# LargeWorldModel/LWM

Measured on AMD Instinct MI355X. Metric: tokens/sec fwd+bwd, LWM-7B RingAttention hot path (32 layers x 32 heads x 128), higher is better.
Workload: dtype bf16 (f32 logits/softmax/accumulate)

## Files before the change

lwm_amd/csrc/attn_fwd64.h:

```cpp
#pragma once

namespace lwm {

constexpr int kF4BQ = 256;
constexpr int kF4BK = 64;
constexpr int kF4Threads = 256;
constexpr int kF4TileBytes = kF4BK * kRowBytes;
constexpr int kF4OffMeta = 4 * kF4TileBytes;
constexpr int kF4OffScan = kF4OffMeta + 3 * kF4BK * 4;
constexpr int kF4LdsBytes = kF4OffScan + 64;
#ifndef LWM_F4_AHEAD
#define LWM_F4_AHEAD 7
#endif
constexpr int kF4Ahead = LWM_F4_AHEAD;
static_assert(kF4Ahead >= 1 && kF4Ahead <= 7, "prefetch distance in fragments");
constexpr int f4_pre_gap(int j) { return 17 - 2 * kF4Ahead + 2 * j; }
constexpr int kF4G0a = 2, kF4G0b = 8, kF4G1a = 2, kF4G1b = 7, kF4G1c = 12, kF4G2a = 1, kF4G2b = 5, kF4G2c = 9;

struct F4Ctx {
    uint32_t ka[8];
    uint32_t vlo[4], vup[4];
    lds_t lds;
    int tid, lane, hi, wave;
    float thr[2];
    float mref[2];
    float nbase[2];
    float lsum[2];
    float c;
    float thr_on;
};

struct F4Stage {
    uint32_t voff_k[4], voff_v[4];
    const char* kb;
    const char* vb;
    int64_t ktile_bytes, vtile_bytes;
};

template <int N>
LWM_DEVICE void f4_dma(const uint32_t* voff, const char* src, lds_t dst) {
#ifdef LWM_EMU
    for (int j = 0; j < N; ++j) glds_load_b128(src + voff[j], dst + 4096 * j);
#else
    const uint64_t a = (uint64_t)src;
    const uint64_t u = ((uint64_t)(uint32_t)__builtin_amdgcn_readfirstlane((int)(a >> 32)) << 32) |
                       (uint32_t)__builtin_amdgcn_readfirstlane((int)a);
    unsigned keep;
    if (N == 4) {
        asm volatile(
            "s_mov_b32 %0, m0\n\ts_nop 3\n\t"
            "s_mov_b32 m0, %6\n\ts_nop 0\n\tglobal_load_lds_dwordx4 %1, %5\n\t"
            "s_add_u32 m0, m0, 0x1000\n\ts_nop 0\n\tglobal_load_lds_dwordx4 %2, %5\n\t"
            "s_add_u32 m0, m0, 0x1000\n\ts_nop 0\n\tglobal_load_lds_dwordx4 %3, %5\n\t"
            "s_add_u32 m0, m0, 0x1000\n\ts_nop 0\n\tglobal_load_lds_dwordx4 %4, %5\n\t"
            "s_mov_b32 m0, %0"
            : "=&s"(keep)
            : "v"(voff[0]), "v"(voff[1]), "v"(voff[2]), "v"(voff[3]), "s"(u), "s"(dst)
            : "memory", "scc");
    } else {
        asm volatile(
            "s_mov_b32 %0, m0\n\ts_nop 3\n\t"
            "s_mov_b32 m0, %4\n\ts_nop 0\n\tglobal_load_lds_dwordx4 %1, %3\n\t"
            "s_add_u32 m0, m0, 0x1000\n\ts_nop 0\n\tglobal_load_lds_dwordx4 %2, %3\n\t"
            "s_mov_b32 m0, %0"
            : "=&s"(keep)
            : "v"(voff[0]), "v"(voff[1]), "s"(u), "s"(dst)
            : "memory", "scc");
    }
#endif
}

LWM_DEVICE void f4_dma1(uint32_t voff, const char* src, lds_t dst) {
#ifdef LWM_EMU
    glds_load_b128(src + voff, dst);
#else
    const uint64_t a = (uint64_t)src;
    const uint64_t u = ((uint64_t)(uint32_t)__builtin_amdgcn_readfirstlane((int)(a >> 32)) << 32) |
                       (uint32_t)__builtin_amdgcn_readfirstlane((int)a);
    asm volatile("s_mov_b32 m0, %2\n\ts_nop 0\n\tglobal_load_lds_dwordx4 %0, %1" ::"v"(voff), "s"(u), "s"(dst) : "memory");
#endif
}
struct F4Dma {
    const char* k_lo_src;
    const char* k_up_src;
    const char* v_src;
    lds_t k_lo_dst, k_up_dst, v_dst;
};

LWM_DEVICE void f4_stage_offsets(const AttnParams& p, int wave, int lane, int kt, F4Stage& st) {
    const int slot = lane & 15;
    for (int j = 0; j < 4; ++j) {
        const int row = 4 * (wave + 4 * j) + (lane >> 4);
        int krow = kt * kF4BK + row;
        krow = krow < p.Sk ? krow : p.Sk - 1;
        const int rel = krow - kt * kF4BK;
        const int col = (slot ^ swz(row)) << 3;
        st.voff_k[j] = (uint32_t)(((int64_t)rel * p.k_ss + col) * 2);
        st.voff_v[j] = (uint32_t)(((int64_t)rel * p.v_ss + col) * 2);
    }
}

LWM_DEVICE void f4_meta_stage(const AttnParams& p, const F4Ctx& cx, int b, int kt, int buf) {
    if (cx.tid < kF4BK) {
        const int krow = kt * kF4BK + cx.tid;
        const int kr = krow < p.Sk ? krow : p.Sk - 1;
        const uint8_t kvalid = p.key_valid ? p.key_valid[(int64_t)b * p.Sk + kr] : (uint8_t)1;
        const int32_t kseg = p.seg_k ? p.seg_k[(int64_t)b * p.Sk + kr] : 0;
        const bool ok = krow < p.Sk && kvalid != 0;
        lds_write_i32(cx.lds + kF4OffMeta + buf * kF4BK * 4 + cx.tid * 4, ok ? kseg : kSegInvalid);
    }
}

#ifdef LWM_EMU
LWM_DEVICE void f4_mfma_s_first(f32x16& d, bf16x8 a, bf16x8 b) { d = mfma_32x32x16(a, b, zero_f32x16()); }
LWM_DEVICE void f4_mfma_s(f32x16& d, bf16x8 a, bf16x8 b) { d = mfma_32x32x16(a, b, d); }
LWM_DEVICE void f4_mfma_o(f32x16& d, bf16x8 a, bf16x8 b) { d = mfma_32x32x16(a, b, d); }
LWM_DEVICE void f4_mfma_settle() {}
LWM_DEVICE void f4_settle_s(f32x16 (&)[2]) {}
LWM_DEVICE void f4_settle_acc(f32x16 (&)[2][4]) {}
LWM_DEVICE float f4_fma(float x, float c, float d) { return fmaf(x, c, d); }
LWM_DEVICE float f4_exp2(float x) { return exp2f(x); }
LWM_DEVICE uint32_t f4_cvt_pk(float lo, float hi) { return pack_bf16x2(lo, hi); }
LWM_DEVICE void f4_add(float& acc, float x) { acc += x; }
LWM_DEVICE float f4_add2(float a, float b) { return a + b; }
LWM_DEVICE void f4_max3(float& m, float a, float b) { m = fmaxf(fmaxf(m, a), b); }
LWM_DEVICE bf16x8 f4_load_agpr(const bf16_t* g) { return __builtin_bit_cast(bf16x8, global_load_b128(g)); }
LWM_DEVICE void f4_load_agpr_wait(bf16x8 (&)[2][8]) {}
LWM_DEVICE void f4_load_agpr_wait8(bf16x8 (&)[8]) {}
LWM_DEVICE void f4_scale_acc(f32x16& d, float alpha) { d *= alpha; }
#else
LWM_DEVICE void f4_mfma_s_first(f32x16& d, bf16x8 a, bf16x8 b) {
    asm volatile("v_mfma_f32_32x32x16_bf16 %0, %1, %2, 0" : "=&v"(d) : "v"(a), "a"(b));
}
LWM_DEVICE void f4_mfma_s(f32x16& d, bf16x8 a, bf16x8 b) {
    asm volatile("v_mfma_f32_32x32x16_bf16 %0, %1, %2, %0" : "+v"(d) : "v"(a), "a"(b));
}
LWM_DEVICE void f4_mfma_o(f32x16& d, bf16x8 a, bf16x8 b) {
    asm volatile("v_mfma_f32_32x32x16_bf16 %0, %1, %2, %0" : "+a"(d) : "v"(a), "v"(b));
}
LWM_DEVICE void f4_mfma_settle() { asm volatile("s_nop 7\n\ts_nop 7"); }
LWM_DEVICE void f4_settle_s(f32x16 (&s)[2]) { asm volatile("s_nop 7\n\ts_nop 7" : "+v"(s[0]), "+v"(s[1])); }
LWM_DEVICE void f4_settle_acc(f32x16 (&a)[2][4]) {
    asm volatile("s_nop 7\n\ts_nop 7"
                 : "+a"(a[0][0]), "+a"(a[0][1]), "+a"(a[0][2]), "+a"(a[0][3]), "+a"(a[1][0]), "+a"(a[1][1]), "+a"(a[1][2]), "+a"(a[1][3]));
}
LWM_DEVICE float f4_fma(float x, float c, float d) {
    float y;
    asm volatile("v_fma_f32 %0, %1, %2, %3" : "=v"(y) : "v"(x), "v"(c), "v"(d));
    return y;
}
LWM_DEVICE float f4_exp2(float x) {
    float y;
    asm volatile("v_exp_f32 %0, %1" : "=v"(y) : "v"(x));
    return y;
}
LWM_DEVICE uint32_t f4_cvt_pk(float lo, float hi) {
    uint32_t y;
    asm volatile("v_cvt_pk_bf16_f32 %0, %1, %2" : "=v"(y) : "v"(lo), "v"(hi));
    return y;
}
LWM_DEVICE void f4_add(float& acc, float x) { asm volatile("v_add_f32 %0, %0, %1" : "+v"(acc) : "v"(x)); }
LWM_DEVICE float f4_add2(float a, float b) {
    float y;
    asm volatile("v_add_f32 %0, %1, %2" : "=v"(y) : "v"(a), "v"(b));
    return y;
}
LWM_DEVICE bf16x8 f4_load_agpr(const bf16_t* g) {
    u32x4 r;
    asm volatile("global_load_dwordx4 %0, %1, off" : "=a"(r) : "v"(g) : "memory");
    return __builtin_bit_cast(bf16x8, r);
}
LWM_DEVICE void f4_load_agpr_wait(bf16x8 (&q)[2][8]) {
    asm volatile("s_waitcnt vmcnt(0)"
                 : "+a"(q[0][0]), "+a"(q[0][1]), "+a"(q[0][2]), "+a"(q[0][3]), "+a"(q[0][4]), "+a"(q[0][5]), "+a"(q[0][6]), "+a"(q[0][7]),
                   "+a"(q[1][0]), "+a"(q[1][1]), "+a"(q[1][2]), "+a"(q[1][3]), "+a"(q[1][4]), "+a"(q[1][5]), "+a"(q[1][6]), "+a"(q[1][7])
                 :
                 : "memory");
}
LWM_DEVICE void f4_load_agpr_wait8(bf16x8 (&q)[8]) {
    asm volatile("s_waitcnt vmcnt(0)"
                 : "+a"(q[0]), "+a"(q[1]), "+a"(q[2]), "+a"(q[3]), "+a"(q[4]), "+a"(q[5]), "+a"(q[6]), "+a"(q[7])
                 :
                 : "memory");
}
LWM_DEVICE void f4_scale_acc(f32x16& d, float alpha) {
#define LWM_F4_SC(i) "v_accvgpr_read_b32 %16, %" #i "\n\ts_nop 0\n\tv_mul_f32 %16, %16, %17\n\ts_nop 0\n\tv_accvgpr_write_b32 %" #i ", %16\n\t"
    float t;
    asm volatile(LWM_F4_SC(0) LWM_F4_SC(1) LWM_F4_SC(2) LWM_F4_SC(3) LWM_F4_SC(4) LWM_F4_SC(5) LWM_F4_SC(6) LWM_F4_SC(7)
                 LWM_F4_SC(8) LWM_F4_SC(9) LWM_F4_SC(10) LWM_F4_SC(11) LWM_F4_SC(12) LWM_F4_SC(13) LWM_F4_SC(14) LWM_F4_SC(15) "s_nop 1"
                 : "+a"(d[0]), "+a"(d[1]), "+a"(d[2]), "+a"(d[3]), "+a"(d[4]), "+a"(d[5]), "+a"(d[6]), "+a"(d[7]),
                   "+a"(d[8]), "+a"(d[9]), "+a"(d[10]), "+a"(d[11]), "+a"(d[12]), "+a"(d[13]), "+a"(d[14]), "+a"(d[15]), "=&v"(t)
                 : "v"(alpha));
#undef LWM_F4_SC
}
LWM_DEVICE void f4_max3(float& m, float a, float b) { asm volatile("v_max3_f32 %0, %0, %1, %2" : "+v"(m) : "v"(a), "v"(b)); }
#endif

template <int KHALF>
LWM_DEVICE bf16x8 f4_kread(const F4Ctx& cx, int s) { return lds_read_b128(cx.ka[s] + KHALF * 32 * kRowBytes); }
template <int VHALF>
LWM_DEVICE bf16x8 f4_vread(const F4Ctx& cx, int f) {
    const uint32_t off = VHALF * 32 * kRowBytes + 16 * (f >> 2) * kRowBytes;
    bf16x4 lo = lds_read_tr16(cx.vlo[f & 3] + off);
    bf16x4 up = lds_read_tr16(cx.vup[f & 3] + off);
    bf16x8 o;
    o[0] = lo[0]; o[1] = lo[1]; o[2] = lo[2]; o[3] = lo[3];
    o[4] = up[0]; o[5] = up[1]; o[6] = up[2]; o[7] = up[3];
    return o;
}

template <int KHALF, bool DO_S, bool DO_FIN, int VNEXT, int DMA>
LWM_DEVICE void f4_phase1(const F4Ctx& cx, const bf16x8 (&qf)[2][8], f32x16 (&sN)[2], float (&tC)[2][16], float (&ps)[2][8],
                          bf16x8 (&pb)[2][2], bf16x8 (&kfr)[8], bf16x8 (&vfr)[8], const F4Stage& st, const F4Dma& dm) {
    uint32_t w[4];
#pragma unroll
    for (int g = 0; g < 16; ++g) {
        const int s = g >> 1, qb = g & 1;
        if (DO_S && qb == 0 && s + kF4Ahead < 8) kfr[s + kF4Ahead] = f4_kread<KHALF>(cx, s + kF4Ahead);
#pragma unroll
        for (int j = 0; j < kF4Ahead; ++j)
            if (VNEXT >= 0 && g == f4_pre_gap(j)) vfr[j] = f4_vread<VNEXT < 0 ? 0 : VNEXT>(cx, j);
        sched_fence();
        if (DO_S) {
            if (s == 0) f4_mfma_s_first(sN[qb], kfr[0], qf[qb][0]);
            else f4_mfma_s(sN[qb], kfr[s], qf[qb][s]);
        }
        if (DMA == 0 && g == kF4G0a) f4_dma1(st.voff_k[2], dm.k_up_src, dm.k_up_dst);
        if (DMA == 0 && g == kF4G0b) f4_dma1(st.voff_k[3], dm.k_up_src, dm.k_up_dst + 4096);
        if (DMA == 2 && g == kF4G2a) f4_dma1(st.voff_v[3], dm.v_src, dm.v_dst + 12288);
        if (DMA == 2 && g == kF4G2b) f4_dma1(st.voff_k[0], dm.k_lo_src, dm.k_lo_dst);
        if (DMA == 2 && g == kF4G2c) f4_dma1(st.voff_k[1], dm.k_lo_src, dm.k_lo_dst + 4096);
        if (DO_FIN) {
            const int e = 2 * g, fq = e >> 4, r = e & 15;
            tC[fq][r] = f4_exp2(tC[fq][r]);
            tC[fq][r + 1] = f4_exp2(tC[fq][r + 1]);
            if (g > 0) {
                const int e0 = 2 * (g - 1), q0 = e0 >> 4, r0 = e0 & 15;
                w[(g - 1) & 3] = f4_cvt_pk(tC[q0][r0], tC[q0][r0 + 1]);
                ps[q0][r0 >> 1] = f4_add2(tC[q0][r0], tC[q0][r0 + 1]);
                if (((g - 1) & 3) == 3) pb[q0][(e0 >> 3) & 1] = __builtin_bit_cast(bf16x8, u32x4{w[0], w[1], w[2], w[3]});
            }
        }
        sched_fence();
    }
    if (DO_FIN) {
        w[3] = f4_cvt_pk(tC[1][14], tC[1][15]);
        ps[1][7] = f4_add2(tC[1][14], tC[1][15]);
        pb[1][1] = __builtin_bit_cast(bf16x8, u32x4{w[0], w[1], w[2], w[3]});
    }
}

template <int VHALF, bool DO_PV, bool DO_MAX, int KNEXT, int DMA>
LWM_DEVICE void f4_phase2(F4Ctx& cx, const bf16x8 (&pb)[2][2], f32x16 (&acc)[2][4], const float (&ps)[2][8],
                          const f32x16 (&sN)[2], float (&tN)[2][16], float (&mx)[2], bf16x8 (&kfr)[8], bf16x8 (&vfr)[8],
                          const F4Stage& st, const F4Dma& dm) {
    float ls[2] = {0.f, 0.f};
    float mp[2] = {-INFINITY, -INFINITY};
#pragma unroll
    for (int h = 0; h < 16; ++h) {
        const int f = h >> 1, qb = h & 1, t = f >> 2, db = f & 3;
        if (DO_PV && qb == 0 && f + kF4Ahead < 8) vfr[f + kF4Ahead] = f4_vread<VHALF>(cx, f + kF4Ahead);
#pragma unroll
        for (int j = 0; j < kF4Ahead; ++j)
            if (KNEXT >= 0 && h == f4_pre_gap(j)) kfr[j] = f4_kread<KNEXT < 0 ? 0 : KNEXT>(cx, j);
        sched_fence();
        if (DO_PV) f4_mfma_o(acc[qb][db], vfr[f], pb[qb][t]);
        if (DMA == 1 && h == kF4G1a) f4_dma1(st.voff_v[0], dm.v_src, dm.v_dst);
        if (DMA == 1 && h == kF4G1b) f4_dma1(st.voff_v[1], dm.v_src, dm.v_dst + 4096);
        if (DMA == 1 && h == kF4G1c) f4_dma1(st.voff_v[2], dm.v_src, dm.v_dst + 8192);
        const int e = 2 * h, fq = e >> 4, r = e & 15;
        if (DO_PV) f4_add(ls[fq], ps[fq][r >> 1]);
        if (DO_MAX) {
            f4_max3(mp[fq], sN[fq][r], sN[fq][r + 1]);
            tN[fq][r] = f4_fma(sN[fq][r], cx.c, cx.nbase[fq]);
            tN[fq][r + 1] = f4_fma(sN[fq][r + 1], cx.c, cx.nbase[fq]);
        }
        sched_fence();
    }
    if (DO_PV)
        for (int q2 = 0; q2 < 2; ++q2) cx.lsum[q2] += ls[q2];
    if (DO_MAX)
        for (int q2 = 0; q2 < 2; ++q2) mx[q2] = mp[q2];
}

template <bool HAS_META, int KHALF>
LWM_DEVICE void f4_mask(const F4Ctx& cx, f32x16 (&sN)[2], const int (&rel)[2], const int32_t (&seg_q)[2], int mbuf) {
#pragma unroll
    for (int qb = 0; qb < 2; ++qb) {
        const int relh = rel[qb] - 4 * cx.hi - 32 * KHALF;
#pragma unroll
        for (int g = 0; g < 4; ++g) {
            if (HAS_META) {
                const u32x4 sg = lds_read_u32x4(cx.lds + kF4OffMeta + mbuf * kF4BK * 4 + 16 * cx.hi + (32 * KHALF + 8 * g) * 4);
#pragma unroll
                for (int j = 0; j < 4; ++j) {
                    const bool vis = ((int32_t)sg[j] == seg_q[qb]) && (8 * g + j <= relh);
                    sN[qb][4 * g + j] = vis ? sN[qb][4 * g + j] : -INFINITY;
                }
            } else {
#pragma unroll
                for (int j = 0; j < 4; ++j) sN[qb][4 * g + j] = (8 * g + j <= relh) ? sN[qb][4 * g + j] : -INFINITY;
            }
        }
    }
}

LWM_DEVICE void f4_rescale(F4Ctx& cx, const float (&mx)[2], f32x16 (&acc)[2][4], float (&tN)[2][16]) {
    f4_settle_acc(acc);
#pragma unroll
    for (int qb = 0; qb < 2; ++qb) {
        const float mxa = fmaxf(mx[qb], xhalf(mx[qb]));
        const float m_new = fmaxf(cx.mref[qb], mxa);
        const float ms = (m_new == -INFINITY) ? 0.0f : m_new;
        const float alpha = fast_exp2((cx.mref[qb] - ms) * cx.c);
        cx.lsum[qb] *= alpha;
        for (int db = 0; db < 4; ++db) f4_scale_acc(acc[qb][db], alpha);
        const float nb_new = -ms * cx.c;
        const float dt = nb_new - cx.nbase[qb];
        for (int r = 0; r < 16; ++r) tN[qb][r] += dt;
        cx.mref[qb] = m_new;
        cx.nbase[qb] = nb_new;
        cx.thr[qb] = (m_new == -INFINITY) ? -INFINITY : m_new + cx.thr_on;
    }
}

template <bool HAS_META>
LWM_DEVICE void attn_fwd64_body(const AttnParams& p) {
    const lds_t lds = dyn_lds();
    const int tid = thread_idx();
    const int wave = wave_uniform(tid >> 6), lane = tid & 63, l31 = lane & 31, hi = lane >> 5;

    const int nqt = (p.Sq + kF4BQ - 1) / kF4BQ;
    const int HB = p.H * p.B;
    int lin = block_idx_x(), qt, hb;
    if ((HB & 7) == 0) {
        int xcd = lin & 7, i = lin >> 3;
        hb = xcd + 8 * (i / nqt);
        qt = nqt - 1 - (i % nqt);
    } else {
        hb = lin / nqt;
        qt = nqt - 1 - (lin % nqt);
    }
    const int b = hb / p.H, h = hb % p.H;
    const bf16_t* qb_ = p.q + (int64_t)b * p.q_sb + (int64_t)h * p.q_sh;

    F4Ctx cx;
    cx.lds = lds;
    cx.tid = tid;
    cx.lane = lane;
    cx.hi = hi;
    cx.wave = wave;
    for (int s = 0; s < 8; ++s) cx.ka[s] = lds + tile_off(l31, 2 * s + hi);
    {
        const TrFragAddr t = frag_tr_addr(lds + 2 * kF4TileBytes, lane);
        for (int db = 0; db < 4; ++db) {
            cx.vlo[db] = t.lo[db];
            cx.vup[db] = t.up[db];
        }
    }
    cx.c = p.scale * kLog2e;
    cx.thr_on = kDeferLog2 / cx.c;

    bf16x8 qf[2][8];
    int q_row[2];
    bool q_ok[2];
    int32_t seg_q[2];
    int64_t q_pos[2];
    const PosMap km = k_map(p);
    const PosTab kt_ = load_postab(km);
    const int64_t q_base = pos_base(load_postab(q_map(p)), qt * kF4BQ);
#pragma unroll
    for (int qb = 0; qb < 2; ++qb) {
        q_row[qb] = qt * kF4BQ + wave * 64 + 32 * qb + l31;
        q_ok[qb] = q_row[qb] < p.Sq;
        q_pos[qb] = q_base + q_row[qb];
        seg_q[qb] = (HAS_META && q_ok[qb] && p.seg_q) ? p.seg_q[(int64_t)b * p.Sq + q_row[qb]] : 0;
        const int qr = q_ok[qb] ? q_row[qb] : p.Sq - 1;
        for (int s = 0; s < 8; ++s) qf[qb][s] = f4_load_agpr(qb_ + (int64_t)qr * p.q_ss + 16 * s + 8 * hi);
        cx.thr[qb] = -INFINITY;
        cx.mref[qb] = -INFINITY;
        cx.nbase[qb] = 0.0f;
        cx.lsum[qb] = 0.0f;
    }
    const int64_t wq_min = q_base + (int64_t)qt * kF4BQ + wave * 64;
    const int64_t wq_max = wq_min + 63;

    const int nkt_all = (p.Sk + kF4BK - 1) / kF4BK;
    int nkt = nkt_all, kt0 = 0;
    const int q_last = (qt * kF4BQ + kF4BQ < p.Sq ? qt * kF4BQ + kF4BQ : p.Sq) - 1;
    if (p.causal) nkt = tiles_reaching(kt_, kF4BK, nkt_all, q_base + q_last);
    if (HAS_META && p.segb_q && p.segb_k && nkt > 0) {
        const int nbq = (p.Sq + 31) >> 5, nbk = (p.Sk + 31) >> 5;
        int smin, smax, lo, hi2;
        seg_own_range(p.segb_q + (int64_t)b * nbq * 2, nbq, qt * (kF4BQ / 32), kF4BQ / 32, smin, smax);
        seg_narrow<kF4Threads>(p.segb_k + (int64_t)b * nbk * 2, nbk, kF4BK / 32, 0, nkt, smin, smax, lds + kF4OffScan, tid, lo, hi2);
        kt0 = lo > 0 ? lo - 1 : 0;
        nkt = hi2;
    }
    const int n_wg = nkt > kt0 ? nkt - kt0 : 0;
    int n_w = n_wg;
    if (p.causal) {
        const int nw = tiles_reaching(kt_, kF4BK, nkt_all, wq_max) - kt0;
        n_w = nw < 0 ? 0 : (nw < n_wg ? nw : n_wg);
    }
    if (wave_uniform(qt * kF4BQ + wave * 64 >= p.Sq ? 1 : 0)) n_w = 0;

    f32x16 acc[2][4];
    for (int qb = 0; qb < 2; ++qb)
        for (int i = 0; i < 4; ++i) acc[qb][i] = zero_f32x16();

    if (n_wg > 0) {
        F4Stage st;
        st.kb = (const char*)(p.k + (int64_t)b * p.k_sb + (int64_t)h * p.k_sh);
        st.vb = (const char*)(p.v + (int64_t)b * p.v_sb + (int64_t)h * p.v_sh);
        st.ktile_bytes = (int64_t)kF4BK * p.k_ss * 2;
        st.vtile_bytes = (int64_t)kF4BK * p.v_ss * 2;
        const bool ragged = (p.Sk % kF4BK) != 0;
        f4_stage_offsets(p, wave, lane, 0, st);
        const lds_t kdst0 = lds + (uint32_t)wave * 1024, vdst0 = lds + 2 * kF4TileBytes + (uint32_t)wave * 1024;
        auto stage_k = [&](int rel, int half) {
            const int kt = kt0 + rel;
            const lds_t dst = kdst0 + (rel & 1) * kF4TileBytes + half * 8192;
            if (ragged && kt == nkt_all - 1) {
                F4Stage s2 = st;
                f4_stage_offsets(p, wave, lane, kt, s2);
                f4_dma<2>(s2.voff_k + 2 * half, st.kb + kt * st.ktile_bytes, dst);
            } else {
                f4_dma<2>(st.voff_k + 2 * half, st.kb + kt * st.ktile_bytes, dst);
            }
        };
        auto stage_v = [&](int rel) {
            const int kt = kt0 + rel;
            const lds_t dst = vdst0 + (rel & 1) * kF4TileBytes;
            if (ragged && kt == nkt_all - 1) {
                F4Stage s2 = st;
                f4_stage_offsets(p, wave, lane, kt, s2);
                f4_dma<4>(s2.voff_v, st.vb + kt * st.vtile_bytes, dst);
            } else {
                f4_dma<4>(st.voff_v, st.vb + kt * st.vtile_bytes, dst);
            }
        };
        auto stage_iter = [&](int i) {
            if (i + 2 < n_wg) stage_k(i + 2, 0);
            if (i + 1 < n_wg) {
                stage_k(i + 1, 1);
                stage_v(i + 1);
            }
            if (HAS_META && i + 2 < n_wg) f4_meta_stage(p, cx, b, kt0 + i + 2, (i + 2) % 3);
        };
        PosCursor kc = cursor_begin(kt_);
        auto rel_of = [&](int rel, int (&r)[2]) {
            const int krow0 = (kt0 + rel) * kF4BK;
            cursor_seek(km, kc, krow0);
            const int64_t k_pos0 = kc.base + krow0;
            for (int qb = 0; qb < 2; ++qb) {
                const int64_t d = p.causal ? (q_pos[qb] - k_pos0) : (int64_t)kF4BK;
                r[qb] = d > kF4BK ? kF4BK : (d < -1 ? -1 : (int)d);
            }
        };
        int first_mask = 0x7fffffff;
        if (p.causal) {
            const int ft = tiles_below(kt_, kF4BK, nkt_all, wq_min) - kt0;
            first_mask = ft < 0 ? 0 : ft;
        }
        auto needs_causal = [&](int rel) -> bool { return rel >= first_mask; };
        const int32_t own_seg = wave_uniform(seg_q[0]);
        const bool own_uniform = HAS_META && !wave_any((q_ok[0] && seg_q[0] != own_seg) || (q_ok[1] && seg_q[1] != own_seg));
        auto meta_words = [&](int mbuf) -> lds_t { return cx.lds + kF4OffMeta + mbuf * kF4BK * 4; };
        bool uni_c = false;
#define LWM_F4_MASK(KHALF_, s_, rel_, mbuf_, uni_, SETTLE_)                                                          \
    do {                                                                                                            \
        if ((HAS_META && !(uni_)) || needs_causal(rel_)) {                                                          \
            int r_[2];                                                                                              \
            if (SETTLE_) f4_settle_s(s_);             \
            rel_of(rel_, r_);                                                                                       \
            if (HAS_META && !(uni_)) f4_mask<HAS_META, KHALF_>(cx, s_, r_, seg_q, mbuf_);                           \
            else f4_mask<false, KHALF_>(cx, s_, r_, seg_q, mbuf_);                                                  \
        }                                                                                                           \
    } while (0)

        stage_k(0, 0);
        stage_k(0, 1);
        stage_v(0);
        if (n_wg > 1) stage_k(1, 0);
        if (HAS_META) {
            f4_meta_stage(p, cx, b, kt0, 0);
            if (n_wg > 1) f4_meta_stage(p, cx, b, kt0 + 1, 1);
        }
        f4_load_agpr_wait(qf);
        block_sync();

        f32x16 sA[2], sB[2];
        float tt[2][16], ps[2][8];
        bf16x8 pb[2][2];
        float mx[2];
        for (int qb = 0; qb < 2; ++qb) {
            sA[qb] = zero_f32x16();
            sB[qb] = zero_f32x16();
            for (int r = 0; r < 16; ++r) tt[qb][r] = 0.0f;
            for (int r = 0; r < 8; ++r) ps[qb][r] = 0.0f;
            for (int t = 0; t < 2; ++t) pb[qb][t] = zero_bf16x8();
        }
        bf16x8 kfr[8], vfr[8];
        for (int j = 0; j < 8; ++j) {
            kfr[j] = zero_bf16x8();
            vfr[j] = zero_bf16x8();
        }
        F4Dma dm = {};
        if (n_w > 0) {
            for (int j = 0; j < kF4Ahead; ++j) kfr[j] = f4_kread<0>(cx, j);
            f4_phase1<0, true, false, -1, -1>(cx, qf, sA, tt, ps, pb, kfr, vfr, st, dm);
            f4_settle_s(sA);
            uni_c = HAS_META && seg_step_uniform(seg_step_word(meta_words(0), lane), own_uniform, own_seg);
            LWM_F4_MASK(0, sA, 0, 0, uni_c, false);
            f4_phase2<0, false, true, -1, -1>(cx, pb, acc, ps, sA, tt, mx, kfr, vfr, st, dm);
            if (wave_any(mx[0] > cx.thr[0] || mx[1] > cx.thr[1])) f4_rescale(cx, mx, acc, tt);
        }
        block_sync();

        int32_t ktog = kF4TileBytes, vtog = kF4TileBytes;
        auto toggle_k = [&]() {
            for (int s = 0; s < 8; ++s) cx.ka[s] += (uint32_t)ktog;
            ktog = -ktog;
        };
        auto toggle_v = [&]() {
            for (int db = 0; db < 4; ++db) {
                cx.vlo[db] += (uint32_t)vtog;
                cx.vup[db] += (uint32_t)vtog;
            }
            vtog = -vtog;
        };
#ifdef LWM_PROF
        unsigned long long f4p[10] = {0, 0, 0, 0, 0, 0, 0, 0, 0, 0}, f4t = __builtin_amdgcn_s_memtime();
        const unsigned long long f4t0 = f4t;
#define F4_LAP(slot)                                                  \
    do {                                                              \
        const unsigned long long now_ = __builtin_amdgcn_s_memtime(); \
        f4p[slot] += now_ - f4t;                                      \
        f4t = now_;                                                   \
    } while (0)
#else
#define F4_LAP(slot)
#endif
#define LWM_F4_TILE(i, D0, D1, D2, D3)                                                                             \
    do {                                                                                                            \
        const int32_t segw_ = HAS_META ? seg_step_word(meta_words(((i) + 1) % 3), lane) : 0;       \
        f4_phase1<1, true, true, 0, D0>(cx, qf, sB, tt, ps, pb, kfr, vfr, st, dm);      \
        F4_LAP(0);                                                                                                  \
        LWM_F4_MASK(1, sB, i, (i) % 3, uni_c, true);                                                                \
        uni_c = HAS_META && seg_step_uniform(segw_, own_uniform, own_seg);                                          \
        toggle_k();                                                                                                 \
        F4_LAP(1);                                                                                                  \
        f4_phase2<0, true, true, 0, D1>(cx, pb, acc, ps, sB, tt, mx, kfr, vfr, st, dm);               \
        if (wave_any(mx[0] > cx.thr[0] || mx[1] > cx.thr[1])) f4_rescale(cx, mx, acc, tt);                          \
        F4_LAP(2);                                                                                                  \
        f4_phase1<0, true, true, 1, D2>(cx, qf, sA, tt, ps, pb, kfr, vfr, st, dm);    \
        F4_LAP(3);                                                                                                  \
        LWM_F4_MASK(0, sA, (i) + 1, ((i) + 1) % 3, uni_c, true);                                                    \
        F4_LAP(4);                                                                                                  \
        f4_phase2<1, true, true, -1, D3>(cx, pb, acc, ps, sA, tt, mx, kfr, vfr, st, dm);            \
        if (wave_any(mx[0] > cx.thr[0] || mx[1] > cx.thr[1])) f4_rescale(cx, mx, acc, tt);                          \
        toggle_v();                                                                                                 \
        F4_LAP(5);                                                                                                  \
        glds_wait_all();                                                                                            \
        F4_LAP(6);                                                                                                  \
        block_sync();                                                                                               \
        F4_LAP(7);                                                                                                  \
    } while (0)
        const int n_hot = n_w > 0 ? n_w - 1 : 0;
        int n_fast = n_hot < n_wg - 2 ? n_hot : n_wg - 2;
        if (ragged && n_fast > nkt_all - 1 - kt0 - 2) n_fast = nkt_all - 1 - kt0 - 2;
        if (n_fast < 0) n_fast = 0;
        int i = 0;
        for (; i < n_fast; ++i) {
            for (int j = 0; j < kF4Ahead; ++j) kfr[j] = f4_kread<1>(cx, j);
            dm.k_lo_src = st.kb + (kt0 + i + 2) * st.ktile_bytes;
            dm.k_up_src = st.kb + (kt0 + i + 1) * st.ktile_bytes;
            dm.v_src = st.vb + (kt0 + i + 1) * st.vtile_bytes;
            dm.k_lo_dst = kdst0 + (i & 1) * kF4TileBytes;
            dm.k_up_dst = kdst0 + ((i + 1) & 1) * kF4TileBytes + 8192;
            dm.v_dst = vdst0 + ((i + 1) & 1) * kF4TileBytes;
            if (HAS_META) f4_meta_stage(p, cx, b, kt0 + i + 2, (i + 2) % 3);
            LWM_F4_TILE(i, 0, 1, 2, -1);
#ifdef LWM_PROF
            f4p[8] += 1;
#endif
        }
#ifdef LWM_PROF
        if (!HAS_META && hb == 0 && qt == nqt - 1 && lane == 0 && p.out_acc) {
            f4p[9] = __builtin_amdgcn_s_memtime() - f4t0;
            for (int j = 0; j < 10; ++j) ((unsigned long long*)p.out_acc)[wave * 10 + j] = f4p[j];
        }
#endif
        for (; i < n_hot; ++i) {
            for (int j = 0; j < kF4Ahead; ++j) kfr[j] = f4_kread<1>(cx, j);
            stage_iter(i);
            LWM_F4_TILE(i, -1, -1, -1, -1);
        }
#undef LWM_F4_TILE
#undef F4_LAP
        if (n_w > 0) {
            for (int j = 0; j < kF4Ahead; ++j) kfr[j] = f4_kread<1>(cx, j);
            stage_iter(i);
            f4_phase1<1, true, true, 0, -1>(cx, qf, sB, tt, ps, pb, kfr, vfr, st, dm);
            LWM_F4_MASK(1, sB, i, i % 3, uni_c, true);
#undef LWM_F4_MASK
            f4_phase2<0, true, true, -1, -1>(cx, pb, acc, ps, sB, tt, mx, kfr, vfr, st, dm);
            if (wave_any(mx[0] > cx.thr[0] || mx[1] > cx.thr[1])) f4_rescale(cx, mx, acc, tt);
            f4_phase1<0, false, true, 1, -1>(cx, qf, sA, tt, ps, pb, kfr, vfr, st, dm);
            f4_phase2<1, true, false, -1, -1>(cx, pb, acc, ps, sA, tt, mx, kfr, vfr, st, dm);
            glds_wait_all();
            block_sync();
            ++i;
        }
        for (; i < n_wg; ++i) {
            stage_iter(i);
            glds_wait_all();
            block_sync();
        }
    }

    if (n_wg <= 0) f4_load_agpr_wait(qf);
    f4_settle_acc(acc);
    const bool carry = p.carry_in != 0, fin = p.final_out != 0;
#pragma unroll
    for (int qb = 0; qb < 2; ++qb) {
        const float l_tot = cx.lsum[qb] + xhalf(cx.lsum[qb]);
        float inv = 0.0f, lse_b = -INFINITY;
        if (l_tot > 0.0f) {
            inv = 1.0f / l_tot;
            lse_b = cx.mref[qb] * p.scale + logf(l_tot);
        }
        float w_a = 0.0f, w_b = 1.0f, lse_new = lse_b;
        const int64_t lse_idx = ((int64_t)b * p.H + h) * p.Sq + q_row[qb];
        if (carry && q_ok[qb]) {
            const float lse_a = p.lse_acc[lse_idx];
            const float mxl = fmaxf(lse_a, lse_b);
            if (mxl == -INFINITY) {
                lse_new = -INFINITY;
                w_a = 0.0f;
                w_b = 0.0f;
            } else {
                const float ea = expf(lse_a - mxl), eb = expf(lse_b - mxl);
                lse_new = mxl + logf(ea + eb);
                w_a = ea / (ea + eb);
                w_b = eb / (ea + eb);
            }
        }
        if (q_ok[qb]) {
            const float sc = inv * w_b;
            bf16_t* const op = p.out + (int64_t)b * p.o_sb + (int64_t)q_row[qb] * p.o_ss + (int64_t)h * p.o_sh + 4 * hi;
            float* const ap = p.out_acc + (((int64_t)b * p.Sq + q_row[qb]) * p.H + h) * kHeadDim + 4 * hi;
            if (fin && !carry) {
#pragma unroll
                for (int db = 0; db < 4; ++db)
#pragma unroll
                    for (int rq = 0; rq < 4; ++rq)
                        global_store_b64(op + 32 * db + 8 * rq,
                                         u32x2{pack_bf16x2(acc[qb][db][4 * rq + 0] * sc, acc[qb][db][4 * rq + 1] * sc),
                                               pack_bf16x2(acc[qb][db][4 * rq + 2] * sc, acc[qb][db][4 * rq + 3] * sc)});
            } else {
#pragma unroll
                for (int db = 0; db < 4; ++db)
#pragma unroll
                    for (int rq = 0; rq < 4; ++rq) {
                        const int d0 = 32 * db + 8 * rq;
                        float o0 = acc[qb][db][4 * rq + 0] * sc, o1 = acc[qb][db][4 * rq + 1] * sc;
                        float o2 = acc[qb][db][4 * rq + 2] * sc, o3 = acc[qb][db][4 * rq + 3] * sc;
                        if (carry) {
                            const f32x4 a = global_load_f32x4(ap + d0);
                            o0 += a[0] * w_a; o1 += a[1] * w_a; o2 += a[2] * w_a; o3 += a[3] * w_a;
                        }
                        if (fin) global_store_b64(op + d0, u32x2{pack_bf16x2(o0, o1), pack_bf16x2(o2, o3)});
                        else global_store_f32x4(ap + d0, f32x4{o0, o1, o2, o3});
                    }
            }
            if (hi == 0) {
                if (fin) p.lse[lse_idx] = lse_new;
                else p.lse_acc[lse_idx] = lse_new;
            }
        }
    }
}

LWM_KERNEL(kF4Threads) void attn_fwd64_kernel(AttnParams p) { attn_fwd64_body<false>(p); }
LWM_KERNEL(kF4Threads) void attn_fwd64_meta_kernel(AttnParams p) { attn_fwd64_body<true>(p); }

}
```

Before: 30720.

## Replace split K/V double buffer with four-slot LDS ring and partial vmem waits

```diff
diff --git a/lwm_amd/csrc/attn_fwd64.h b/lwm_amd/csrc/attn_fwd64.h
--- a/lwm_amd/csrc/attn_fwd64.h
+++ b/lwm_amd/csrc/attn_fwd64.h
@@ -6,16 +6,22 @@
 constexpr int kF4BK = 64;
 constexpr int kF4Threads = 256;
 constexpr int kF4TileBytes = kF4BK * kRowBytes;
-constexpr int kF4OffMeta = 4 * kF4TileBytes;
-constexpr int kF4OffScan = kF4OffMeta + 3 * kF4BK * 4;
+constexpr int kF4Slots = 4;
+constexpr int kF4SlotBytes = 2 * kF4TileBytes;
+constexpr int kF4OffMeta = kF4Slots * kF4SlotBytes;
+constexpr int kF4OffScan = kF4OffMeta + kF4Slots * kF4BK * 4;
 constexpr int kF4LdsBytes = kF4OffScan + 64;
+static_assert(kF4LdsBytes <= 160 * 1024, "one workgroup per CU, 160 KiB of LDS");
+static_assert((kF4Slots & (kF4Slots - 1)) == 0, "slot = tile & (kF4Slots - 1)");
+constexpr int kF4PiecesPerTile = 8;
 #ifndef LWM_F4_AHEAD
 #define LWM_F4_AHEAD 7
 #endif
 constexpr int kF4Ahead = LWM_F4_AHEAD;
 static_assert(kF4Ahead >= 1 && kF4Ahead <= 7, "prefetch distance in fragments");
 constexpr int f4_pre_gap(int j) { return 17 - 2 * kF4Ahead + 2 * j; }
-constexpr int kF4G0a = 2, kF4G0b = 8, kF4G1a = 2, kF4G1b = 7, kF4G1c = 12, kF4G2a = 1, kF4G2b = 5, kF4G2c = 9;
+constexpr int kF4PiecePhase[8] = {0, 0, 1, 1, 1, 2, 2, 2};
+constexpr int kF4PieceGap[8] = {2, 8, 2, 7, 12, 1, 5, 9};
 
 struct F4Ctx {
     uint32_t ka[8];
@@ -81,11 +87,29 @@
 #endif
 }
 struct F4Dma {
-    const char* k_lo_src;
-    const char* k_up_src;
+    const char* k_src;
     const char* v_src;
-    lds_t k_lo_dst, k_up_dst, v_dst;
+    lds_t k_dst, v_dst;
 };
+template <int PHASE>
+LWM_DEVICE void f4_dma_gap(int gap, const F4Stage& st, const F4Dma& dm) {
+#pragma unroll
+    for (int j = 0; j < 8; ++j)
+        if (PHASE == kF4PiecePhase[j] && gap == kF4PieceGap[j]) {
+            if (j < 4) f4_dma1(st.voff_k[j], dm.k_src, dm.k_dst + 4096 * j);
+            else f4_dma1(st.voff_v[j - 4], dm.v_src, dm.v_dst + 4096 * (j - 4));
+        }
+}
+
+LWM_DEVICE void f4_ring_barrier() {
+#ifdef LWM_EMU
+    block_sync_lds();
+#else
+    asm volatile("" ::: "memory");
+    __builtin_amdgcn_s_barrier();
+    asm volatile("" ::: "memory");
+#endif
+}
 
 LWM_DEVICE void f4_stage_offsets(const AttnParams& p, int wave, int lane, int kt, F4Stage& st) {
     const int slot = lane & 15;
@@ -225,11 +249,7 @@
             if (s == 0) f4_mfma_s_first(sN[qb], kfr[0], qf[qb][0]);
             else f4_mfma_s(sN[qb], kfr[s], qf[qb][s]);
         }
-        if (DMA == 0 && g == kF4G0a) f4_dma1(st.voff_k[2], dm.k_up_src, dm.k_up_dst);
-        if (DMA == 0 && g == kF4G0b) f4_dma1(st.voff_k[3], dm.k_up_src, dm.k_up_dst + 4096);
-        if (DMA == 2 && g == kF4G2a) f4_dma1(st.voff_v[3], dm.v_src, dm.v_dst + 12288);
-        if (DMA == 2 && g == kF4G2b) f4_dma1(st.voff_k[0], dm.k_lo_src, dm.k_lo_dst);
-        if (DMA == 2 && g == kF4G2c) f4_dma1(st.voff_k[1], dm.k_lo_src, dm.k_lo_dst + 4096);
+        f4_dma_gap<DMA>(g, st, dm);
         if (DO_FIN) {
             const int e = 2 * g, fq = e >> 4, r = e & 15;
             tC[fq][r] = f4_exp2(tC[fq][r]);
@@ -265,9 +285,7 @@
             if (KNEXT >= 0 && h == f4_pre_gap(j)) kfr[j] = f4_kread<KNEXT < 0 ? 0 : KNEXT>(cx, j);
         sched_fence();
         if (DO_PV) f4_mfma_o(acc[qb][db], vfr[f], pb[qb][t]);
-        if (DMA == 1 && h == kF4G1a) f4_dma1(st.voff_v[0], dm.v_src, dm.v_dst);
-        if (DMA == 1 && h == kF4G1b) f4_dma1(st.voff_v[1], dm.v_src, dm.v_dst + 4096);
-        if (DMA == 1 && h == kF4G1c) f4_dma1(st.voff_v[2], dm.v_src, dm.v_dst + 8192);
+        f4_dma_gap<DMA>(h, st, dm);
         const int e = 2 * h, fq = e >> 4, r = e & 15;
         if (DO_PV) f4_add(ls[fq], ps[fq][r >> 1]);
         if (DO_MAX) {
@@ -352,7 +370,7 @@
     cx.wave = wave;
     for (int s = 0; s < 8; ++s) cx.ka[s] = lds + tile_off(l31, 2 * s + hi);
     {
-        const TrFragAddr t = frag_tr_addr(lds + 2 * kF4TileBytes, lane);
+        const TrFragAddr t = frag_tr_addr(lds + kF4TileBytes, lane);
         for (int db = 0; db < 4; ++db) {
             cx.vlo[db] = t.lo[db];
             cx.vup[db] = t.up[db];
@@ -417,36 +435,25 @@
         st.vtile_bytes = (int64_t)kF4BK * p.v_ss * 2;
         const bool ragged = (p.Sk % kF4BK) != 0;
         f4_stage_offsets(p, wave, lane, 0, st);
-        const lds_t kdst0 = lds + (uint32_t)wave * 1024, vdst0 = lds + 2 * kF4TileBytes + (uint32_t)wave * 1024;
-        auto stage_k = [&](int rel, int half) {
+        const lds_t kdst0 = lds + (uint32_t)wave * 1024, vdst0 = lds + kF4TileBytes + (uint32_t)wave * 1024;
+        auto stage_tile = [&](int rel) {
             const int kt = kt0 + rel;
-            const lds_t dst = kdst0 + (rel & 1) * kF4TileBytes + half * 8192;
+            const uint32_t slot = (uint32_t)(rel & (kF4Slots - 1)) * kF4SlotBytes;
             if (ragged && kt == nkt_all - 1) {
                 F4Stage s2 = st;
                 f4_stage_offsets(p, wave, lane, kt, s2);
-                f4_dma<2>(s2.voff_k + 2 * half, st.kb + kt * st.ktile_bytes, dst);
+                f4_dma<4>(s2.voff_k, st.kb + kt * st.ktile_bytes, kdst0 + slot);
+                f4_dma<4>(s2.voff_v, st.vb + kt * st.vtile_bytes, vdst0 + slot);
             } else {
-                f4_dma<2>(st.voff_k + 2 * half, st.kb + kt * st.ktile_bytes, dst);
-            }
-        };
-        auto stage_v = [&](int rel) {
-            const int kt = kt0 + rel;
-            const lds_t dst = vdst0 + (rel & 1) * kF4TileBytes;
-            if (ragged && kt == nkt_all - 1) {
-                F4Stage s2 = st;
-                f4_stage_offsets(p, wave, lane, kt, s2);
-                f4_dma<4>(s2.voff_v, st.vb + kt * st.vtile_bytes, dst);
-            } else {
-                f4_dma<4>(st.voff_v, st.vb + kt * st.vtile_bytes, dst);
+                f4_dma<4>(st.voff_k, st.kb + kt * st.ktile_bytes, kdst0 + slot);
+                f4_dma<4>(st.voff_v, st.vb + kt * st.vtile_bytes, vdst0 + slot);
             }
         };
         auto stage_iter = [&](int i) {
-            if (i + 2 < n_wg) stage_k(i + 2, 0);
-            if (i + 1 < n_wg) {
-                stage_k(i + 1, 1);
-                stage_v(i + 1);
-            }
-            if (HAS_META && i + 2 < n_wg) f4_meta_stage(p, cx, b, kt0 + i + 2, (i + 2) % 3);
+            if (i + 3 < n_wg) {
+                if (HAS_META) f4_meta_stage(p, cx, b, kt0 + i + 3, (i + 3) & (kF4Slots - 1));
+                stage_tile(i + 3);
+            }
         };
         PosCursor kc = cursor_begin(kt_);
         auto rel_of = [&](int rel, int (&r)[2]) {
@@ -479,14 +486,11 @@
         }                                                                                                           \
     } while (0)
 
-        stage_k(0, 0);
-        stage_k(0, 1);
-        stage_v(0);
-        if (n_wg > 1) stage_k(1, 0);
-        if (HAS_META) {
-            f4_meta_stage(p, cx, b, kt0, 0);
-            if (n_wg > 1) f4_meta_stage(p, cx, b, kt0 + 1, 1);
-        }
+        for (int t = 0; t < kF4Slots - 1; ++t)
+            if (t < n_wg) {
+                if (HAS_META) f4_meta_stage(p, cx, b, kt0 + t, t);
+                stage_tile(t);
+            }
         f4_load_agpr_wait(qf);
         block_sync();
 
@@ -513,22 +517,23 @@
             f4_settle_s(sA);
             uni_c = HAS_META && seg_step_uniform(seg_step_word(meta_words(0), lane), own_uniform, own_seg);
             LWM_F4_MASK(0, sA, 0, 0, uni_c, false);
-            f4_phase2<0, false, true, -1, -1>(cx, pb, acc, ps, sA, tt, mx, kfr, vfr, st, dm);
+            f4_phase2<0, false, true, 1, -1>(cx, pb, acc, ps, sA, tt, mx, kfr, vfr, st, dm);
             if (wave_any(mx[0] > cx.thr[0] || mx[1] > cx.thr[1])) f4_rescale(cx, mx, acc, tt);
         }
-        block_sync();
-
-        int32_t ktog = kF4TileBytes, vtog = kF4TileBytes;
-        auto toggle_k = [&]() {
-            for (int s = 0; s < 8; ++s) cx.ka[s] += (uint32_t)ktog;
-            ktog = -ktog;
+
+        auto ring_step = [&](int i) -> uint32_t {
+            return ((i + 1) & (kF4Slots - 1)) ? (uint32_t)kF4SlotBytes : (uint32_t)(-(kF4Slots - 1) * kF4SlotBytes);
         };
-        auto toggle_v = [&]() {
+        auto advance_k = [&](int i) {
+            const uint32_t d = ring_step(i);
+            for (int s = 0; s < 8; ++s) cx.ka[s] += d;
+        };
+        auto advance_v = [&](int i) {
+            const uint32_t d = ring_step(i);
             for (int db = 0; db < 4; ++db) {
-                cx.vlo[db] += (uint32_t)vtog;
-                cx.vup[db] += (uint32_t)vtog;
-            }
-            vtog = -vtog;
+                cx.vlo[db] += d;
+                cx.vup[db] += d;
+            }
         };
 #ifdef LWM_PROF
         unsigned long long f4p[10] = {0, 0, 0, 0, 0, 0, 0, 0, 0, 0}, f4t = __builtin_amdgcn_s_memtime();
@@ -542,46 +547,47 @@
 #else
 #define F4_LAP(slot)
 #endif
-#define LWM_F4_TILE(i, D0, D1, D2, D3)                                                                             \
+#define LWM_F4_TILE(i, FAST, D0, D1, D2, D3)                                                                       \
     do {                                                                                                            \
-        const int32_t segw_ = HAS_META ? seg_step_word(meta_words(((i) + 1) % 3), lane) : 0;       \
+        const int32_t segw_ = HAS_META ? seg_step_word(meta_words(((i) + 1) & (kF4Slots - 1)), lane) : 0;       \
         f4_phase1<1, true, true, 0, D0>(cx, qf, sB, tt, ps, pb, kfr, vfr, st, dm);      \
         F4_LAP(0);                                                                                                  \
-        LWM_F4_MASK(1, sB, i, (i) % 3, uni_c, true);                                                                \
+        LWM_F4_MASK(1, sB, i, (i) & (kF4Slots - 1), uni_c, true);                                                   \
         uni_c = HAS_META && seg_step_uniform(segw_, own_uniform, own_seg);                                          \
-        toggle_k();                                                                                                 \
+        advance_k(i);                                                                                               \
         F4_LAP(1);                                                                                                  \
         f4_phase2<0, true, true, 0, D1>(cx, pb, acc, ps, sB, tt, mx, kfr, vfr, st, dm);               \
         if (wave_any(mx[0] > cx.thr[0] || mx[1] > cx.thr[1])) f4_rescale(cx, mx, acc, tt);                          \
         F4_LAP(2);                                                                                                  \
         f4_phase1<0, true, true, 1, D2>(cx, qf, sA, tt, ps, pb, kfr, vfr, st, dm);    \
         F4_LAP(3);                                                                                                  \
-        LWM_F4_MASK(0, sA, (i) + 1, ((i) + 1) % 3, uni_c, true);                                                    \
+        LWM_F4_MASK(0, sA, (i) + 1, ((i) + 1) & (kF4Slots - 1), uni_c, true);                                       \
         F4_LAP(4);                                                                                                  \
-        f4_phase2<1, true, true, -1, D3>(cx, pb, acc, ps, sA, tt, mx, kfr, vfr, st, dm);            \
+         \
+        f4_phase2<1, true, true, 1, D3>(cx, pb, acc, ps, sA, tt, mx, kfr, vfr, st, dm);                             \
         if (wave_any(mx[0] > cx.thr[0] || mx[1] > cx.thr[1])) f4_rescale(cx, mx, acc, tt);                          \
-        toggle_v();                                                                                                 \
+        advance_v(i);                                                                                               \
         F4_LAP(5);                                                                                                  \
-        glds_wait_all();                                                                                            \
+        if (FAST) wait_vmem_le<kF4PiecesPerTile>();                                                                 \
+        else glds_wait_all();                                                                                       \
         F4_LAP(6);                                                                                                  \
-        block_sync();                                                                                               \
+        if (FAST) f4_ring_barrier();                                                                                \
+        else block_sync();                                                                                          \
         F4_LAP(7);                                                                                                  \
     } while (0)
         const int n_hot = n_w > 0 ? n_w - 1 : 0;
-        int n_fast = n_hot < n_wg - 2 ? n_hot : n_wg - 2;
-        if (ragged && n_fast > nkt_all - 1 - kt0 - 2) n_fast = nkt_all - 1 - kt0 - 2;
+        int n_fast = n_hot < n_wg - 3 ? n_hot : n_wg - 3;
+        if (ragged && n_fast > nkt_all - 1 - kt0 - 3) n_fast = nkt_all - 1 - kt0 - 3;
         if (n_fast < 0) n_fast = 0;
         int i = 0;
         for (; i < n_fast; ++i) {
-            for (int j = 0; j < kF4Ahead; ++j) kfr[j] = f4_kread<1>(cx, j);
-            dm.k_lo_src = st.kb + (kt0 + i + 2) * st.ktile_bytes;
-            dm.k_up_src = st.kb + (kt0 + i + 1) * st.ktile_bytes;
-            dm.v_src = st.vb + (kt0 + i + 1) * st.vtile_bytes;
-            dm.k_lo_dst = kdst0 + (i & 1) * kF4TileBytes;
-            dm.k_up_dst = kdst0 + ((i + 1) & 1) * kF4TileBytes + 8192;
-            dm.v_dst = vdst0 + ((i + 1) & 1) * kF4TileBytes;
-            if (HAS_META) f4_meta_stage(p, cx, b, kt0 + i + 2, (i + 2) % 3);
-            LWM_F4_TILE(i, 0, 1, 2, -1);
+            const uint32_t slot = (uint32_t)((i + 3) & (kF4Slots - 1)) * kF4SlotBytes;
+            dm.k_src = st.kb + (kt0 + i + 3) * st.ktile_bytes;
+            dm.v_src = st.vb + (kt0 + i + 3) * st.vtile_bytes;
+            dm.k_dst = kdst0 + slot;
+            dm.v_dst = vdst0 + slot;
+            if (HAS_META) f4_meta_stage(p, cx, b, kt0 + i + 3, (i + 3) & (kF4Slots - 1));
+            LWM_F4_TILE(i, true, 0, 1, 2, 3);
 #ifdef LWM_PROF
             f4p[8] += 1;
 #endif
@@ -593,17 +599,15 @@
         }
 #endif
         for (; i < n_hot; ++i) {
-            for (int j = 0; j < kF4Ahead; ++j) kfr[j] = f4_kread<1>(cx, j);
             stage_iter(i);
-            LWM_F4_TILE(i, -1, -1, -1, -1);
+            LWM_F4_TILE(i, false, -1, -1, -1, -1);
         }
 #undef LWM_F4_TILE
 #undef F4_LAP
         if (n_w > 0) {
-            for (int j = 0; j < kF4Ahead; ++j) kfr[j] = f4_kread<1>(cx, j);
             stage_iter(i);
             f4_phase1<1, true, true, 0, -1>(cx, qf, sB, tt, ps, pb, kfr, vfr, st, dm);
-            LWM_F4_MASK(1, sB, i, i % 3, uni_c, true);
+            LWM_F4_MASK(1, sB, i, i & (kF4Slots - 1), uni_c, true);
 #undef LWM_F4_MASK
             f4_phase2<0, true, true, -1, -1>(cx, pb, acc, ps, sB, tt, mx, kfr, vfr, st, dm);
             if (wave_any(mx[0] > cx.thr[0] || mx[1] > cx.thr[1])) f4_rescale(cx, mx, acc, tt);
```

Result: no change. 30940 (median of 6 runs) (+0.7%).
